# pbs-plus/pbs-plus

Measured on AMD Instinct MI355X. Metric: GiB/s ingested through CDC+SHA-256, higher is better.
Workload: dtype u32

## Files before the change

### include/pbsgpu.h

```cpp
#ifndef PBSGPU_H
#define PBSGPU_H

#include <stddef.h>
#include <stdint.h>

#ifdef __cplusplus
extern "C" {
#endif

#define PBSGPU_ABI_VERSION 5

#define PBSGPU_OK 0
#define PBSGPU_E_INVALID (-1)
#define PBSGPU_E_NO_DEVICE (-2)
#define PBSGPU_E_HIP (-3)
#define PBSGPU_E_NOMEM (-4)
#define PBSGPU_E_CAPACITY (-5)
#define PBSGPU_E_BUSY (-6)
#define PBSGPU_E_TICKET (-7)
#define PBSGPU_E_STATE (-9)

const char *pbsgpu_strerror(int status);
int pbsgpu_abi_version(void);
int pbsgpu_last_hip_error(void);
// ... 145 lines not shown
    uint32_t fill_cus;
    uint32_t reserved1;
    uint64_t reserved[2];
} pbsgpu_ring_options;
#define PBSGPU_RING_OFF 0xffffffffu
#define PBSGPU_RING_F_NO_OVERLAP 1u
#define PBSGPU_RING_F_NO_STAGE 2u
#define PBSGPU_RING_F_NO_CUT_PRIO 4u
#define PBSGPU_RING_F_NO_SPLIT_AUTO 8u
#define PBSGPU_RING_F_DEFER_SERVICE 16u
#define PBSGPU_RING_F_FILL_SERIAL 32u
#define PBSGPU_RING_F_DENSE_SERVICE 64u
#define PBSGPU_RING_F_DENSE_LANES 128u
#define PBSGPU_RING_F_TIER_TAG 256u
#define PBSGPU_RING_F_HOLD_PAGES 512u
typedef struct pbsgpu_ring_stats {
    uint64_t page_bytes, bytes_enqueued, chunks, candidates, pages_enqueued, pages_recycled, service_bytes_last;
    uint32_t pages_total, pages_free, sha_cus, rounds, rounds_done, rounds_in_flight, streams_opened, service_launches;
    double service_ms_last;
    double service_ms_total;
} pbsgpu_ring_stats;
int pbsgpu_ring_create(pbsgpu_engine *eng, const pbsgpu_ring_options *opt , pbsgpu_ring **out);
void pbsgpu_ring_destroy(pbsgpu_ring *ring);
int pbsgpu_ring_open(pbsgpu_ring *ring, uint32_t *stream);
int pbsgpu_ring_reserve(pbsgpu_ring *ring, uint32_t stream, void **dptr, uint64_t *cap);
int pbsgpu_ring_commit(pbsgpu_ring *ring, uint32_t stream, uint64_t nbytes, int final);
int pbsgpu_ring_fill(pbsgpu_ring *ring, uint32_t stream, uint64_t seed, uint32_t kind, uint64_t nbytes, int final,
                     uint64_t *taken);
typedef struct pbsgpu_fill_piece {
    uint64_t dst_off;
// ... 297 lines not shown
```

### pbs_plus_amd/_lib.py

```python
from __future__ import annotations

import ctypes as C
import os
import subprocess

import numpy as np

_HERE = os.path.dirname(os.path.abspath(__file__))
LIB_PATH = os.environ.get("PBSGPU_LIB_PATH") or os.path.join(_HERE, "lib", "libpbsgpu.so")
CSRC = os.path.join(_HERE, "csrc")

OK = 0
E_INVALID, E_NO_DEVICE, E_HIP, E_NOMEM, E_CAPACITY, E_BUSY, E_TICKET, _E_RETIRED_8, E_STATE = range(-1, -10, -1)


class PbsGpuError(RuntimeError):
    def __init__(self, status: int, what: str = ""):
        self.status = status
        msg = lib().pbsgpu_strerror(status).decode() if _lib is not None else str(status)
        hip = lib().pbsgpu_last_hip_error() if _lib is not None else 0
        extra = ""
        if _lib is not None and ("comm" in what or "allgather" in what):
            txt = lib().pbsgpu_comm_last_error()
            if txt:
# ... 44 lines not shown

class ReuseChunk(C.Structure):
    _fields_ = [("size", C.c_uint64), ("padding", C.c_uint64), ("end_offset", C.c_uint64), ("digest", C.c_uint8 * 32)]


class FileHash(C.Structure):
    _fields_ = [("index", C.c_uint64), ("size", C.c_uint64), ("xxh3", C.c_uint64)]


RING_OFF = 0xFFFFFFFF
RING_F_NO_OVERLAP, RING_F_NO_STAGE, RING_F_NO_CUT_PRIO, RING_F_NO_SPLIT_AUTO, RING_F_DEFER_SERVICE, RING_F_FILL_SERIAL = 1, 2, 4, 8, 16, 32
RING_F_DENSE_SERVICE = 64
RING_F_DENSE_LANES = 128
RING_F_TIER_TAG = 256
RING_F_HOLD_PAGES = 512
RING_ANY_STREAM = 0xFFFFFFFF


class RingOptions(C.Structure):
    _fields_ = [("arena_bytes", C.c_uint64), ("page_bytes", C.c_uint64), ("max_streams", C.c_uint32),
                ("sha_cus", C.c_uint32), ("round_pages", C.c_uint32), ("express_cus", C.c_uint32),
                ("min_round_pages", C.c_uint32), ("max_inflight", C.c_uint32), ("long_bytes", C.c_uint32),
                ("long_lo_bytes", C.c_uint32), ("long_spill", C.c_uint32), ("poll_every", C.c_uint32), ("flags", C.c_uint32),
                ("lanes_cus", C.c_uint32), ("backlog_mib", C.c_double), ("lone_defer_ms", C.c_double),
                ("idle_timeout_s", C.c_double), ("autopark_ms", C.c_double), ("short_bytes", C.c_uint64), ("fill_cus", C.c_uint32),
                ("reserved1", C.c_uint32), ("reserved", C.c_uint64 * 2)]


class EngineOptions(C.Structure):
    _fields_ = [("inflight", C.c_uint32), ("sha_form", C.c_uint32), ("sha_slack_pct", C.c_uint32), ("sha_dense_pct", C.c_uint32),
# ... 246 lines not shown
```

### pbs_plus_amd/csrc/kernels.h

```cpp
#pragma once

#include <hip/hip_runtime.h>
#include <stdint.h>

#include "../../include/pbsgpu.h"

namespace pbsk {

constexpr int kWindow = 64;

struct ScanParams {
    const uint8_t *data_al;
    uint32_t lead;
    uint64_t nbytes;
    uint64_t ntiles;
    uint32_t tile_bytes;
    const uint32_t *table_rot;
    uint32_t thr;
    uint32_t cap;
    uint32_t *tile_cnt;
    uint32_t *tile_slots;
    unsigned long long *tile_queue;
    uint32_t tiles_per_wave;
    uint32_t shared_chip;
// ... 117 lines not shown
        unsigned long long lq;
    };
    uint32_t head;
    uint32_t free_count;
    uint32_t error;
    uint32_t rounds_done;
    uint32_t xp_busy;
    uint32_t pad0;
    union {
        struct {
            uint32_t stail;
            uint32_t shead;
        };
        unsigned long long sq;
    };
    uint32_t pad[4];
};
static_assert(sizeof(RingCtl) == 64, "RingCtl is one 64-byte line");
struct RingDesc {
    uint64_t p1, p2v;
    uint32_t len, len1, cell, pages;
};
__host__ __device__ inline void ring_desc_encode(uint4 *q, const uint32_t slot, const RingDesc &d) {
    q[2u * slot] = make_uint4((uint32_t)d.p1, (uint32_t)(d.p1 >> 32), d.len, d.len1);
    q[2u * slot + 1u] = make_uint4((uint32_t)d.p2v, (uint32_t)(d.p2v >> 32), d.cell, d.pages);
}
__host__ __device__ inline RingDesc ring_desc_decode(const uint4 e0, const uint4 e1) {
    return RingDesc{((uint64_t)e0.y << 32) | e0.x, ((uint64_t)e1.y << 32) | e1.x, e0.z, e0.w, e1.z, e1.w};
}

constexpr uint32_t kCellBytes = 64;
// ... 15 lines not shown
    uint32_t smask;
    uint32_t short_bytes;
    uint32_t short_room;
    RingCtl *ctl;
    uint8_t *cells;
    uint32_t *pending;
    unsigned long long *free_fifo;
    uint32_t free_mask;
    const uint32_t *heartbeat;
    unsigned long long idle_ticks;
    uint32_t poll_mask;
    uint32_t xp;
    uint32_t long_spill;
    uint32_t xp_pairs;
    uint32_t long_lo;
};
constexpr int kHbBeat = 0, kHbIntent = 16, kHbCommitted = 17, kHbClaim = 32, kHbRoundsEnq = 33;
constexpr uint32_t kRingProbeSteps = 4096;


enum : int { kRsNcand = 0, kRsNrec = 1, kRsMaxcnt = 2, kRsNlong = 3, kRsNshort = 4, kRsShortRoom = 5, kRsTileq = 6 , kRsNmain = 8, kRsCount = 10 };

struct RingPage {
    uint64_t phys_off;
    uint64_t logical;
    uint32_t valid;
    uint32_t slot;
    uint32_t phys;
    uint32_t seg;
    uint64_t fill_seed;
    uint64_t fill_off;
// ... 107 lines not shown
```

### pbs_plus_amd/csrc/kernels.hip

```cpp
#include "kernel_util.h"
#include "kernels.h"
#include "ring_queue.h"

namespace pbsk {

__device__ __forceinline__ uint32_t rotr(uint32_t x, int n) { return __builtin_rotateright32(x, n); }

__device__ __forceinline__ uint32_t xor3(uint32_t a, uint32_t b, uint32_t c) {
    return __builtin_amdgcn_bitop3_b32(a, b, c, 0x96);
}
__device__ __forceinline__ uint32_t maj3(uint32_t a, uint32_t b, uint32_t c) {
    return __builtin_amdgcn_bitop3_b32(a, b, c, 0xE8);
}
__device__ __forceinline__ uint32_t ch3(uint32_t e, uint32_t f, uint32_t g) { return g ^ (e & (f ^ g)); }

__device__ constexpr uint32_t kSha256K[64] = {
    0x428a2f98, 0x71374491, 0xb5c0fbcf, 0xe9b5dba5, 0x3956c25b, 0x59f111f1, 0x923f82a4, 0xab1c5ed5,
    0xd807aa98, 0x12835b01, 0x243185be, 0x550c7dc3, 0x72be5d74, 0x80deb1fe, 0x9bdc06a7, 0xc19bf174,
    0xe49b69c1, 0xefbe4786, 0x0fc19dc6, 0x240ca1cc, 0x2de92c6f, 0x4a7484aa, 0x5cb0a9dc, 0x76f988da,
    0x983e5152, 0xa831c66d, 0xb00327c8, 0xbf597fc7, 0xc6e00bf3, 0xd5a79147, 0x06ca6351, 0x14292967,
    0x27b70a85, 0x2e1b2138, 0x4d2c6dfc, 0x53380d13, 0x650a7354, 0x766a0abb, 0x81c2c92e, 0x92722c85,
    0xa2bfe8a1, 0xa81a664b, 0xc24b8b70, 0xc76c51a3, 0xd192e819, 0xd6990624, 0xf40e3585, 0x106aa070,
    0x19a4c116, 0x1e376c08, 0x2748774c, 0x34b0bcb5, 0x391c0cb3, 0x4ed8aa4a, 0x5b9cca4f, 0x682e6ff3,
    0x748f82ee, 0x78a5636f, 0x84c87814, 0x8cc70208, 0x90befffa, 0xa4506ceb, 0xbef9a3f7, 0xc67178f2};
// ... 362 lines not shown
        constexpr int D = 2;
        uint32_t R[D][17];
        uint32_t selv[D], cflag[D];
        uint8_t *dstv[D];
        [[maybe_unused]] uint32_t pagesv[D];
#pragma unroll
        for (int s = 0; s < D; ++s) {
#pragma unroll
            for (int j = 0; j < 17; ++j) R[s][j] = 0;
            selv[s] = 0x00010203u;
            cflag[s] = 0;
            dstv[s] = nullptr;
            pagesv[s] = 0xffffffffu;
        }

        constexpr uint32_t kReserve = 16;
        uint32_t res_next = 0, res_end = 0;
        [[maybe_unused]] uint32_t poll_ctr = 0;
        auto acquire = [&](bool need) {
            if constexpr (Source::kRing) {
                if (__ballot(need) == 0) return;
                if (__ballot(have) != 0 && ((++poll_ctr) & src.poll_mask) != 0u) return;
                const bool long_only = src.long_bytes != 0u && src.xp == 0u && (lane & 15) == 0;
                const bool elig = need && claimed == 0u;
                if (src.long_bytes && __ballot(elig)) {
                    uint32_t lh;
                    int32_t avail = ring_queue_avail(&src.ctl->lq, lh) - (int32_t)src.long_spill;
                    if (avail > 0 && src.xp != 0u && (uint32_t)avail <= src.xp_pairs &&
                        __hip_atomic_load(&src.ctl->xp_busy, __ATOMIC_RELAXED, __HIP_MEMORY_SCOPE_AGENT) < src.xp_pairs)
                        avail = 0;
// ... 77 lines not shown
                    exhausted = true;
                    have = false;
                }
            }
            if constexpr (DENSE) {
                const uint32_t cnt = (uint32_t)__popcll(m);
                if (cnt > avail) {
                    res_next = first + (cnt - avail);
                    res_end = res_next + kReserve;
                } else {
                    res_next += cnt;
                }
            }
        };
        auto prep = [&](const int s) {
            acquire(!have && !exhausted);
            uint32_t c = 0;
            const uint8_t *p = reinterpret_cast<const uint8_t *>(kIdleBlock);
            const uint8_t *bb = base;
            uint64_t off = 0;
            bool tail = false, last = false;
            if (have) {
                off = blk * 64;
                if constexpr (Source::kRing) bb = (off < len1) ? base : base2;
                last = blk + 1 == nblk;
                if (off + 64 <= len) p = bb + off;
                else tail = true;
                c = 1u | (last ? 2u : 0u);
                dstv[s] = dst;
                if constexpr (Source::kRing) pagesv[s] = pages;
// ... 113 lines not shown
        auto rounds = [&](const Blk &x) {
            if (x.c & 1u) {
                uint32_t a = H[0], b = H[1], cc = H[2], dd = H[3], e = H[4], f = H[5], g = H[6], h = H[7];
#pragma unroll
                for (int q = 0; q < 16; q += 2) {
                    SHA256_ROUND(a, b, cc, dd, e, f, g, h, x.wk[q].x);
                    SHA256_ROUND(h, a, b, cc, dd, e, f, g, x.wk[q].y);
                    SHA256_ROUND(g, h, a, b, cc, dd, e, f, x.wk[q].z);
                    SHA256_ROUND(f, g, h, a, b, cc, dd, e, x.wk[q].w);
                    SHA256_ROUND(e, f, g, h, a, b, cc, dd, x.wk[q + 1].x);
                    SHA256_ROUND(dd, e, f, g, h, a, b, cc, x.wk[q + 1].y);
                    SHA256_ROUND(cc, dd, e, f, g, h, a, b, x.wk[q + 1].z);
                    SHA256_ROUND(b, cc, dd, e, f, g, h, a, x.wk[q + 1].w);
                }
                H[0] += a; H[1] += b; H[2] += cc; H[3] += dd; H[4] += e; H[5] += f; H[6] += g; H[7] += h;
                if (x.c & 2u) {
                    PBSK_GLOBAL uint32_t *o = (PBSK_GLOBAL uint32_t *)x.d;
#pragma unroll
                    for (int j = 0; j < 8; ++j) o[j] = __builtin_bswap32(H[j]);
                    if constexpr (Source::kRing) ring_cell_publish(o);
                    sha256_iv(H);
                }
            }
        };
        Blk A, B;
        __syncthreads();
        fetch(A, 0);
        for (;;) {
            if (!A.al) break;
            __syncthreads();
            fetch(B, 1);
            __builtin_amdgcn_sched_barrier(0);
            rounds(A);
            if (!B.al) break;
            __syncthreads();
// ... 77 lines not shown
    auto any_alive = [&](const int pb) -> uint32_t { return alive[0][pb] | alive[1][pb]; };
    for (int i = threadIdx.x; i < 2 * 2 * 2 * 16 * 32; i += 256) {
        const int row = 2 * (i & 31) + 1, q = (i >> 5) & 15, pl = (i >> 9) & 1, pb = (i >> 10) & 1, pp = (i >> 11) & 1;
        wkbuf_[pp][pb][pl][q][row] = make_uint4(1u, 1u, 1u, 1u);
    }
    __syncthreads();

    if (producer) {
        const uint32_t nitems = nitems_p ? *nitems_p : nitems_imm;
        const uint8_t *base = nullptr;
        uint64_t len = 0, blk = 0, nblk = 0;
        uint8_t *dst = nullptr;
        bool have = false, exhausted = false;
        [[maybe_unused]] const uint8_t *base2 = nullptr;
        [[maybe_unused]] uint32_t len1 = 0, pages = 0xffffffffu;
        [[maybe_unused]] unsigned long long idle_since = 0;
        [[maybe_unused]] uint32_t poll_ctr = 0;
        constexpr int D = 2;
        uint32_t R[D][17];
        uint32_t selv[D], cflag[D];
        uint8_t *dstv[D];
        [[maybe_unused]] uint32_t pagesv[D];
#pragma unroll
        for (int s = 0; s < D; ++s) {
#pragma unroll
            for (int j = 0; j < 17; ++j) R[s][j] = 0;
            selv[s] = 0x00010203u;
            cflag[s] = 0;
            dstv[s] = nullptr;
            pagesv[s] = 0xffffffffu;
        }
        auto acquire = [&](bool need) {
            if (__ballot(need) == 0) return;
            bool got = false;
            if constexpr (Source::kRing) {
                if (__ballot(have) != 0 && ((++poll_ctr) & src.poll_mask) != 0u) return;
                uint32_t lh;
                const int32_t avail = ring_queue_avail(&src.ctl->lq, lh);
                const unsigned long long mn = __ballot(need);
                if (avail > 0) {
                    const uint32_t cnt = min((uint32_t)__popcll(mn), (uint32_t)avail);
                    const uint32_t first = ring_cas_claim(&src.ctl->lhead, lh, cnt, mn, lane);
                    if (first != 0xffffffffu) {
                        const uint32_t rank = wave_rank(mn, lane);
                        got = need && rank < cnt;
                        uint4 e0, e1;
                        ring_desc_load(src.ldesc, (first + rank) & src.lmask, got, e0, e1);
                        ring_desc_take(src, got, e0, e1, base, base2, len, len1, dst, pages);
                        if (lane == __ffsll((long long)mn) - 1) atomicAdd(&src.ctl->xp_busy, cnt);
                    }
                } else if (ring_stop_raised(src) && ring_drained_after_stop(&src.ctl->lq)) {
                    exhausted = exhausted | need;
                }
            } else {
                const unsigned long long m = __ballot(need);
                const uint32_t first = wave_claim(queue, m, (uint32_t)__popcll(m), lane);
                if (need) {
                    const uint32_t i = first + wave_rank(m, lane);
                    if (i < nitems) {
                        src.get(i, base, len, dst);
                        got = true;
                    } else {
                        exhausted = true;
                    }
                }
            }
            const int srcl = lane & ~1;
// ... 9 lines not shown
                    dst = reinterpret_cast<uint8_t *>(ds);
                }
                if constexpr (Source::kRing) {
                    const uint64_t b2 = (uint64_t)__shfl((unsigned long long)reinterpret_cast<uintptr_t>(base2), srcl, 64);
                    const uint32_t l1 = (uint32_t)__shfl((int)len1, srcl, 64);
                    const uint32_t pg = (uint32_t)__shfl((int)pages, srcl, 64);
                    if (pgot) {
                        base2 = reinterpret_cast<const uint8_t *>(b2);
                        len1 = l1;
                        pages = pg;
                    }
                }
                if (pgot) {
                    nblk = (len + 8) / 64 + 1;
                    blk = roleB ? 1ull : 0ull;
                    have = blk < nblk;
                }
            }
        };
        auto prep = [&](const int s) {
            const unsigned long long hm = __ballot(have);
            const bool pair_busy = ((hm >> (lane & ~1)) & 3ull) != 0ull;
            acquire(!roleB && !pair_busy && !exhausted);
            uint32_t c = 0;
            const uint8_t *p = reinterpret_cast<const uint8_t *>(kIdleBlock);
            const uint8_t *bb = base;
            uint64_t off = 0;
            bool tail = false, last = false;
            if (have) {
                off = blk * 64;
                if constexpr (Source::kRing) bb = (off < len1) ? base : base2;
                last = blk + 1 == nblk;
                if (off + 64 <= len) p = bb + off;
                else tail = true;
                c = 1u | (last ? 2u : 0u);
                dstv[s] = dst;
                if constexpr (Source::kRing) pagesv[s] = pages;
                blk += 2;
                if (blk >= nblk) have = false;
            }
            sha256_request_block(p, R[s], selv[s]);
            if (tail) {
                sha256_tail_words(bb, len, off, last, R[s]);
                selv[s] = 0x00010203u;
            }
            cflag[s] = c;
        };
        const int wrow = lane & ~1, wplane = lane & 1;

#pragma unroll
        for (int s = 0; s < D; ++s) prep(s);
        bool drained = false;
// ... 63 lines not shown
        uint32_t HR[4] = {ivr[0], ivr[1], ivr[2], ivr[3]};
        struct Blk {
            uint32_t al, c;
            uint8_t *d;
            uint4 wk[16];
        };
        auto fetch = [&](Blk &x, const int pb, const int plane) {
            x.al = any_alive(pb);
            x.c = ctrl[pb][plane][ci];
            x.d = dstp[pb][plane][ci];
#pragma unroll
            for (int q = 0; q < 16; ++q) x.wk[q] = wkbuf[pb][plane][q][lane];
        };
        auto rounds = [&](const Blk &x) {
            if (x.c & 1u) {
                uint32_t x0 = xp_sel(role, HR[0], HR[2]), x1 = xp_sel(role, HR[1], HR[3]), x2 = HR[2], x3 = HR[3];
                xp_round4<true>(x0, x1, x2, x3, x.wk[0], R, HR[1], HR[0]);
#pragma unroll
                for (int g = 1; g < 16; ++g) xp_round4<false>(x0, x1, x2, x3, x.wk[g], R);
                const uint32_t o63 = x0, o62 = x1, o61 = x2, o60 = x3;
                xp_round2(x0, x1, x2, x3, x.wk[15].w, R);
                HR[0] += xp_sel(role, o63, x0);
                HR[1] += xp_sel(role, o62, x1);
                HR[2] += xp_sel(role, o61, o63);
                HR[3] += xp_sel(role, o60, o62);
                if (x.c & 2u) {
                    PBSK_GLOBAL uint32_t *o = (PBSK_GLOBAL uint32_t *)x.d + (roleB ? 0 : 4);
#pragma unroll
                    for (int j = 0; j < 4; ++j) o[j] = __builtin_bswap32(HR[j]);
                    if constexpr (Source::kRing) ring_cell_publish((PBSK_GLOBAL uint32_t *)x.d);
// ... 207 lines not shown
```

### pbs_plus_amd/csrc/ring.cpp

```cpp
#include <chrono>
#include <cstdio>
#include <cstdlib>
#include <thread>

#include "ring_internal.h"

using namespace pbse;

namespace {

double now_ms() {
    return std::chrono::duration<double, std::milli>(std::chrono::steady_clock::now().time_since_epoch()).count();
}

volatile uint32_t *hb_words(const pbsgpu_ring *r) { return r->heartbeat.as<volatile uint32_t>(); }

void ring_service_ended(pbsgpu_ring *r) {
    if (r->svc == SvcState::Stopped) return;
    r->svc = SvcState::Stopped;
    float ms = 0;
    if (hipEventElapsedTime(&ms, r->ev_svc0, r->ev_svc1) == hipSuccess) {
        r->st.service_ms_last = ms;
        r->st.service_ms_total += ms;
    } else {
// ... 477 lines not shown
        {"PBSGPU_RING_LONG_SPILL", U32, &o.long_spill, 0},
        {"PBSGPU_RING_POLL_EVERY", U32, &o.poll_every, 0},
        {"PBSGPU_RING_BACKLOG_MIB", F64_ZERO_NEG, &o.backlog_mib, 0},
        {"PBSGPU_RING_LONE_DEFER_MS", F64_ZERO_NEG, &o.lone_defer_ms, 0},
        {"PBSGPU_RING_IDLE_TIMEOUT_S", F64, &o.idle_timeout_s, 0},
        {"PBSGPU_RING_AUTOPARK_MS", F64, &o.autopark_ms, 0},
        {"PBSGPU_RING_OVERLAP", FLAG_IF_ZERO, &o.flags, PBSGPU_RING_F_NO_OVERLAP},
        {"PBSGPU_RING_STAGE_INPUTS", FLAG_IF_ZERO, &o.flags, PBSGPU_RING_F_NO_STAGE},
        {"PBSGPU_RING_CUT_PRIO", FLAG_IF_ZERO, &o.flags, PBSGPU_RING_F_NO_CUT_PRIO},
        {"PBSGPU_RING_SPLIT_AUTO", FLAG_IF_ZERO, &o.flags, PBSGPU_RING_F_NO_SPLIT_AUTO},
        {"PBSGPU_RING_DEFER_SERVICE", FLAG_IF_SET, &o.flags, PBSGPU_RING_F_DEFER_SERVICE},
        {"PBSGPU_RING_FILL_SERIAL", FLAG_IF_SET, &o.flags, PBSGPU_RING_F_FILL_SERIAL},
        {"PBSGPU_RING_DENSE_SERVICE", FLAG_IF_SET, &o.flags, PBSGPU_RING_F_DENSE_SERVICE},
        {"PBSGPU_RING_DENSE_LANES", FLAG_IF_SET, &o.flags, PBSGPU_RING_F_DENSE_LANES},
        {"PBSGPU_RING_TIER_TAG", FLAG_IF_SET, &o.flags, PBSGPU_RING_F_TIER_TAG},
    };
    for (const Entry &e : table) {
        const char *v = getenv(e.name);
        if (!v || !*v) continue;
        switch (e.kind) {
        case U32: *static_cast<uint32_t *>(e.field) = (uint32_t)std::max(0L, atol(v)); break;
        case U32_ZERO_OFF: *static_cast<uint32_t *>(e.field) = atol(v) <= 0 ? PBSGPU_RING_OFF : (uint32_t)atol(v); break;
        case U64: *static_cast<uint64_t *>(e.field) = strtoull(v, nullptr, 10); break;
        case F64: *static_cast<double *>(e.field) = std::max(0.0, atof(v)); break;
        case F64_ZERO_NEG: *static_cast<double *>(e.field) = atof(v) <= 0.0 ? -1.0 : atof(v); break;
        case FLAG_IF_ZERO: if (atoi(v) == 0) *static_cast<uint32_t *>(e.field) |= e.flag; break;
        case FLAG_IF_SET: if (atoi(v) != 0) *static_cast<uint32_t *>(e.field) |= e.flag; break;
        }
    }
}
// ... 15 lines not shown
    const pbsp::QueuePolicy pol = pbsp::queue_policy({lanes_cus, xp_cus, dense_lanes, long_lo_auto, long_bytes, opt_long_lo,
                                                      opt_long_spill, opt_poll_every, idle_timeout_s, eng->cfg.max,
                                                      std::min(eng->effmin, eng->cfg.min)});
    q.short_room = pol.short_room;
    q.xp_pairs = pol.xp_pairs;
    q.long_spill = pol.long_spill;
    q.long_lo = pol.long_lo;
    q.idle_ticks = pol.idle_ticks;
    q.poll_mask = pol.poll_mask;
    q.ctl = ctl.as<pbsk::RingCtl>();
    q.cells = cells.as<uint8_t>();
    q.pending = pending.as<uint32_t>();
    q.free_fifo = free_fifo.as<unsigned long long>();
    q.free_mask = nfree - 1;
    q.heartbeat = heartbeat.as<uint32_t>();
    return q;
}

namespace pbse {

void ring_pop_records(pbsgpu_ring *r, uint32_t slot, pbsgpu_record *out, uint64_t cap, uint64_t *n) {
    StreamSlot &s = r->slots[slot];
    const uint8_t *cells = r->cells.as<uint8_t>();
    while (*n < cap && !s.cells.empty()) {
        const CellRef cr = s.cells.front();
        const uint8_t *c = cells + (size_t)cr.cell * pbsk::kCellBytes;
        const volatile uint32_t *cw = reinterpret_cast<const volatile uint32_t *>(c);
        if (cw[pbsk::kCellFlag] != 1u) break;
        std::atomic_thread_fence(std::memory_order_acquire);
        pbsgpu_record rec;
// ... 102 lines not shown
    r->opt_fill_cus = o.fill_cus;
    r->stage_inputs = !(o.flags & PBSGPU_RING_F_NO_STAGE);
    return PBSGPU_OK;
}

static int ring_allocate(pbsgpu_ring *r, bool overlap) {
    const uint64_t ntiles = r->ntiles;
    CHK(r->arena.ensure((size_t)r->npages * r->stride + 512));
    CHK(r->ctl.ensure(256));
    CHK(r->probe.ensure(128));
    CHK(r->streams.ensure((size_t)r->max_streams * sizeof(pbsk::RingStreamState)));
    CHK(r->pending.ensure((size_t)r->npages * 4 + 64));
    CHK(r->desc.ensure((size_t)r->qslots * 32));
    CHK(r->ldesc.ensure((size_t)r->lslots * 32));
    CHK(r->sdesc.ensure((size_t)r->sslots * 32));
    CHK(r->scalars.ensure(pbsk::kRsCount * 4 + 64));
    CHK(r->tile_cnt.ensure((size_t)ntiles * 4 + 16));
    CHK(r->tile_off.ensure((size_t)ntiles * 4 + 16));
    CHK(r->tile_slots.ensure((size_t)ntiles * r->cap * 4 + 16));
    CHK(r->tileq.ensure(128 + kRingInputs * 8));
    if (overlap) {
        CHK(r->tile_cnt2.ensure((size_t)ntiles * 4 + 16));
        CHK(r->tile_slots2.ensure((size_t)ntiles * r->cap * 4 + 16));
    }
    CHK(r->dense.ensure((size_t)r->dense_cap * 8 + 16));
    CHK(r->scan_tmp.ensure(pbsk::scan_tmp_words(std::max<uint64_t>(ntiles, r->max_streams)) * 4 + 64));
    CHK(r->segs.ensure((size_t)r->max_streams * sizeof(pbsgpu_segment)));
    CHK(r->seg_cnt.ensure((size_t)r->max_streams * 4 + 16));
    CHK(r->seg_off.ensure((size_t)r->max_streams * 4 + 16));
    CHK(r->seg_newc.ensure((size_t)r->max_streams * 8 + 16));
// ... 15 lines not shown
    r->input_stride = r->in_status_off + 128;
    CHK(r->inputs.ensure(r->input_stride * kRingInputs));
    if (r->stage_inputs) CHK(r->inputs_dev.ensure(r->input_stride * kRingInputs));
    std::memset(r->inputs.p, 0, r->input_stride * kRingInputs);
    return PBSGPU_OK;
}

static int ring_streams_and_events(pbsgpu_ring *r, bool overlap, bool cut_prio) {
    int prio_lo = 0, prio_hi = 0;
    HIPCHK(hipDeviceGetStreamPriorityRange(&prio_lo, &prio_hi));
    r->bulk_prio = cut_prio ? prio_lo : 0;
    HIPCHK(hipStreamCreateWithFlags(&r->cs, hipStreamNonBlocking));
    HIPCHK(hipStreamCreateWithPriority(&r->fs, hipStreamNonBlocking, r->bulk_prio));
    HIPCHK(hipMemsetAsync(r->ctl.p, 0, 256, r->cs));
    HIPCHK(hipMemsetAsync(r->probe.p, 0, 128, r->cs));
    HIPCHK(hipMemsetAsync(r->streams.p, 0, (size_t)r->max_streams * sizeof(pbsk::RingStreamState), r->cs));
    HIPCHK(hipMemsetAsync(r->pending.p, 0, (size_t)r->npages * 4 + 64, r->cs));
    HIPCHK(hipMemsetAsync(r->scalars.p, 0, pbsk::kRsCount * 4 + 64, r->cs));
    HIPCHK(hipMemsetAsync(r->tileq.p, 0, 128 + kRingInputs * 8, r->cs));
    HIPCHK(hipStreamSynchronize(r->cs));
    for (auto &ev : r->ev_fill) HIPCHK(hipEventCreateWithFlags(&ev, hipEventDisableTiming));
    if (overlap) {
        HIPCHK(hipStreamCreateWithPriority(&r->ps, hipStreamNonBlocking, r->bulk_prio));
        for (auto &ev : r->ev_scan) HIPCHK(hipEventCreateWithFlags(&ev, hipEventDisableTiming));
        for (auto &ev : r->ev_ctl) HIPCHK(hipEventCreateWithFlags(&ev, hipEventDisableTiming));
    }
    HIPCHK(hipStreamCreateWithPriority(&r->ss, hipStreamNonBlocking, prio_hi));
    if (r->xp_cus) {
        HIPCHK(hipStreamCreateWithPriority(&r->xs, hipStreamNonBlocking, prio_hi));
        HIPCHK(hipEventCreateWithFlags(&r->ev_xsvc1, hipEventDisableTiming));
// ... 23 lines not shown
    r->eng = e;
    const bool overlap = !(o.flags & PBSGPU_RING_F_NO_OVERLAP);
    int st = ring_shape(r, o, long_bytes_hint);
    if (st == PBSGPU_OK) st = ring_allocate(r, overlap);
    if (st == PBSGPU_OK) st = ring_streams_and_events(r, overlap, !(o.flags & PBSGPU_RING_F_NO_CUT_PRIO));
    if (st != PBSGPU_OK) {
        pbsgpu_ring_destroy(r);
        return st;
    }
    r->slots.resize(r->max_streams);
    r->piece_tab.resize(r->max_streams);
    r->piece_n.assign(r->max_streams, 0);
    r->free_pages.reserve(r->npages);
    for (uint32_t p = r->npages; p-- > 0;) r->free_pages.push_back(p);
    r->hold = (o.flags & PBSGPU_RING_F_HOLD_PAGES) != 0;
    if (r->hold) r->held.init(r->npages, r->max_streams, r->page_bytes);
    r->st.pages_total = r->npages;
    r->st.page_bytes = r->page_bytes;
    r->st.sha_cus = r->sha_cus;
    *out = r;
    return PBSGPU_OK;
}

}

extern "C" {

int pbsgpu_ring_create(pbsgpu_engine *e, const pbsgpu_ring_options *opt, pbsgpu_ring **out) {
    return ring_create_internal(e, opt, true, out);
}
// ... 64 lines not shown
        if (r->fs) (void)hipStreamDestroy(r->fs);
        for (auto ev : r->ev_scan)
            if (ev) (void)hipEventDestroy(ev);
        for (auto ev : r->ev_ctl)
            if (ev) (void)hipEventDestroy(ev);
        for (auto ev : r->ev_fill)
            if (ev) (void)hipEventDestroy(ev);
        for (hipEvent_t ev : {r->ev_reset, r->ev_svc0, r->ev_svc1})
            if (ev) (void)hipEventDestroy(ev);
        for (auto &s : r->slots)
            for (auto &q : s.ready)
                if (q.dep) r->ev_pool.push_back(q.dep);
        for (auto ev : r->ev_pool) (void)hipEventDestroy(ev);
        for (DevBuf *b : {&r->arena, &r->ctl, &r->probe, &r->streams, &r->pending, &r->desc, &r->ldesc, &r->sdesc, &r->scalars, &r->tile_cnt, &r->tile_off,
                          &r->tile_slots, &r->tile_cnt2, &r->tile_slots2, &r->tileq, &r->scan_tmp, &r->dense, &r->segs, &r->seg_cnt, &r->seg_off, &r->recs, &r->seg_newc,
                          &r->seg_open, &r->seg_ecand_in, &r->seg_ecand, &r->inputs_dev})
            b->release();
        r->cells.release();
        r->heartbeat.release();
        r->free_fifo.release();
        r->inputs.release();
        for (auto &b : r->sugg_in) b.release();
        for (auto &b : r->piece_tab) b.release();
    }
    const bool unref = r->holds_engine_ref;
    delete r;
    if (e && unref) engine_unref(e);
}

int pbsgpu_ring_open(pbsgpu_ring *r, uint32_t *stream) {
    if (!r || !stream) return PBSGPU_E_INVALID;
// ... 454 lines not shown
        const StreamSlot &s = r->slots[i];
        if (!s.open) continue;
        put("stream %u: committed=%llu enqueued=%llu final_committed=%d final_enqueued=%d final_done=%d ready=%zu cells=%zu "
            "out=%llu | device c=%llu end=%llu\n", i, (unsigned long long)s.bytes_committed,
            (unsigned long long)s.bytes_enqueued, (int)s.final_committed, (int)s.final_enqueued, (int)s.final_done,
            s.ready.size(), s.cells.size(), (unsigned long long)s.records_out, (unsigned long long)sts[i].c,
            (unsigned long long)sts[i].end);
        if (!s.cells.empty()) {
            const uint8_t *c = r->cells.as<uint8_t>() + (size_t)s.cells.front().cell * pbsk::kCellBytes;
            pbsgpu_record rec;
            std::memcpy(&rec, c, sizeof(rec));
            put("  waiting for cell %u: end=%llu size=%u flag=%u\n", s.cells.front().cell, (unsigned long long)rec.end, rec.size,
                reinterpret_cast<const uint32_t *>(c)[pbsk::kCellFlag]);
        }
    }
    return PBSGPU_OK;
}

int pbsgpu_ring_express(pbsgpu_ring *r, uint32_t *express_cus, uint64_t *long_bytes) {
    if (!r) return PBSGPU_E_INVALID;
    if (express_cus) *express_cus = r->xp_cus;
    if (long_bytes) *long_bytes = r->xp_cus ? r->long_bytes : 0;
    return PBSGPU_OK;
}

int pbsgpu_ring_get_probe(pbsgpu_ring *r, pbsgpu_ring_probe *out) {
    if (!r || !out) return PBSGPU_E_INVALID;
    static_assert(sizeof(pbsgpu_ring_probe) == 48, "six counters");
    if (r->svc == SvcState::Running) {
        ring_reap_rounds(r);
// ... 24 lines not shown
```

### pbs_plus_amd/csrc/ring_internal.h

```cpp
#pragma once

#include <deque>
#include <mutex>
#include <vector>

#include "engine_internal.h"
#include "hold.h"
#include "ring_plan.h"

namespace pbse {

constexpr uint32_t kRingInputs = 16;
constexpr uint32_t kPagesPerStreamRound = 256;

struct PageReq {
    uint32_t phys = 0;
    uint64_t k = 0;
    uint32_t valid = 0;
    bool final = false;
    bool do_fill = false;
    uint64_t seed = 0, fill_off = 0;
    uint32_t kind = 0;
    const pbsk::FillPiece *tab = nullptr;
    uint32_t ntab = 0;
// ... 37 lines not shown
    uint64_t new_bytes = 0;
};

enum class SvcState { Stopped, Running, Stopping };

}

struct pbsgpu_ring : pbsp::RingShape {
    pbsgpu_engine *eng = nullptr;
    bool holds_engine_ref = true;
    std::mutex mu;
    uint64_t ready_bytes = 0, inflight_bytes = 0;
    uint32_t tail_seen = 0;
    uint64_t pub_positions = 0, pub_bytes = 0;
    pbse::DevBuf arena, ctl, streams, pending, desc, ldesc, sdesc, probe;
    unsigned long long probe_seen[6] = {};
    bool probe_seen_valid = false;
    unsigned long long ctl_phase_ticks[2][5] = {};
    unsigned long long ctl_phase_rounds[2] = {};
    pbse::DevBuf scalars, tile_cnt, tile_off, tile_slots, scan_tmp, dense, segs, seg_cnt, seg_off, recs, seg_newc, seg_open;
    pbse::DevBuf tile_cnt2, tile_slots2, tileq;
    pbse::DevBuf seg_ecand_in, seg_ecand;
    pbse::DevBuf inputs_dev;
    bool stage_inputs = true;
    pbse::PinnedBuf cells, free_fifo, inputs, heartbeat;
    std::vector<pbse::PinnedBuf> piece_tab;
    std::vector<uint32_t> piece_n;
    pbse::PinnedBuf sugg_in[pbse::kRingInputs];
    size_t input_stride = 0, in_pages_off = 0, in_segs_off = 0, in_recbase_off = 0, in_suggidx_off = 0, in_status_off = 0;
    hipStream_t cs = nullptr, ss = nullptr, fs = nullptr;
// ... 102 lines not shown
```

### pbs_plus_amd/csrc/ring_plan.h

```cpp
#pragma once

#include <algorithm>
#include <cstddef>
#include <cstdint>
#include <cstdlib>

#include "../../include/pbsgpu.h"

namespace pbsp {

inline uint32_t pow2_at_least(uint64_t v) {
    uint32_t p = 1;
    while (p < v && p < (1u << 31)) p <<= 1;
    return p;
}

struct ChunkerView {
    uint32_t min, effmin, avg, max, mask;
    uint32_t minsz() const { return std::min(effmin, min); }
};

inline uint64_t seg_cell_bound(uint32_t take, uint64_t page_bytes, uint32_t maxsz, uint32_t minsz) {
    return ((uint64_t)take * page_bytes + maxsz) / minsz + 2;
}
// ... 187 lines not shown
    q.long_lo = (v.xp_cus && v.long_lo_auto) ? (uint32_t)((uint64_t)v.cfg_max * 11 / 16) : 0u;
    if (v.opt_long_lo) q.long_lo = (v.xp_cus && v.opt_long_lo != PBSGPU_RING_OFF) ? v.opt_long_lo : 0u;
    if (q.long_lo >= v.long_bytes) q.long_lo = 0u;
    if (v.opt_long_spill) q.long_spill = v.opt_long_spill;
    const double idle_s = v.idle_timeout_s > 0 ? std::max(0.05, v.idle_timeout_s) : 20.0;
    q.idle_ticks = (unsigned long long)(idle_s * 100e6);
    {
        const uint64_t min_steps = v.minsz / 64u;
        int every = (int)std::min<uint64_t>(64, std::max<uint64_t>(8, pow2_at_least(min_steps / 256u + 1u) / 2u));
        if (v.opt_poll_every) every = (int)v.opt_poll_every;
        q.poll_mask = pow2_at_least((uint64_t)every) - 1u;
    }
    return q;
}

}
```

### pbs_plus_amd/csrc/ring_queue.h

```cpp
#pragma once

#include "kernel_util.h"
#include "kernels.h"

namespace pbsk {


__device__ __forceinline__ uint32_t wave_rank(const unsigned long long m, const int lane) {
    return (uint32_t)__popcll(m & ((1ull << lane) - 1ull));
}

__device__ __forceinline__ uint32_t wave_claim(uint32_t *queue, const unsigned long long m, const uint32_t n, const int lane) {
    uint32_t first = 0;
    const int leader = __ffsll((long long)m) - 1;
    if (lane == leader) first = atomicAdd(queue, n);
    return __shfl(first, leader, 64);
}

__device__ __forceinline__ int32_t ring_queue_avail(const unsigned long long *q, uint32_t &head) {
    const unsigned long long v = __hip_atomic_load(q, __ATOMIC_RELAXED, __HIP_MEMORY_SCOPE_AGENT);
    head = (uint32_t)(v >> 32);
    return (int32_t)((uint32_t)v - head);
}

// ... 25 lines not shown
    len = take ? (uint64_t)d.len : len;
    len1 = take ? d.len1 : len1;
    dst = take ? src.cells + (uint64_t)d.cell * kCellBytes + 4u * kCellDigest : dst;
    pages = take ? d.pages : pages;
}

__device__ __forceinline__ bool ring_drained_after_stop(const unsigned long long *q) {
    __atomic_thread_fence(__ATOMIC_ACQUIRE);
    uint32_t h;
    return ring_queue_avail(q, h) <= 0;
}
__device__ __forceinline__ bool ring_stop_raised(const RingSource &src) {
    return (uint32_t)(__hip_atomic_load(&src.ctl->tail_stop, __ATOMIC_RELAXED, __HIP_MEMORY_SCOPE_AGENT) >> 32) != 0u;
}

__device__ __forceinline__ void ring_report_free(const RingSource &q, const uint32_t page) {
    const uint32_t fs = atomicAdd(&q.ctl->free_count, 1u);
    __hip_atomic_store(&q.free_fifo[fs & q.free_mask], ((unsigned long long)(fs + 1u) << 32) | page, __ATOMIC_RELAXED,
                       __HIP_MEMORY_SCOPE_SYSTEM);
}
__device__ __forceinline__ void ring_release_page(const RingSource &q, const uint32_t page) {
    if (__hip_atomic_fetch_sub(&q.pending[page], 1u, __ATOMIC_RELEASE, __HIP_MEMORY_SCOPE_AGENT) == 1u) ring_report_free(q, page);
}
__device__ __forceinline__ void ring_release_pages(const RingSource &q, const uint32_t pages) {
#pragma unroll
    for (int h = 0; h < 2; ++h) {
        const uint32_t pi = h ? (pages >> 16) : (pages & 0xffffu);
        if (pi != 0xffffu) ring_release_page(q, pi);
    }
}
// ... 8 lines not shown
```

Baseline: 708.7.

## Hand over long in-progress SHA chunks from lane workers to idle express pairs

Adds a continuation queue so single-lane SHA workers can periodically offer a long chunk still in progress, saving their intermediate hash state and remaining descriptor into a cont slot. Idle express-pair (xp) workers claim these entries, reload the saved state and finish the chunk with the faster two-lane path. The aim is to cut tail latency from long chunks that are stuck on slow lanes while xp capacity sits idle. In exchange it adds atomics, fences, extra per-block flag checks and new termination conditions, which raises ordering and correctness risk. It is on by default and can be turned off with a new flag or environment variable.

```diff
diff --git a/include/pbsgpu.h b/include/pbsgpu.h
--- a/include/pbsgpu.h
+++ b/include/pbsgpu.h
@@ -183,6 +183,7 @@
 #define PBSGPU_RING_F_DENSE_LANES 128u
 #define PBSGPU_RING_F_TIER_TAG 256u
 #define PBSGPU_RING_F_HOLD_PAGES 512u
+#define PBSGPU_RING_F_NO_HANDOVER 1024u
 typedef struct pbsgpu_ring_stats {
     uint64_t page_bytes, bytes_enqueued, chunks, candidates, pages_enqueued, pages_recycled, service_bytes_last;
     uint32_t pages_total, pages_free, sha_cus, rounds, rounds_done, rounds_in_flight, streams_opened, service_launches;
diff --git a/pbs_plus_amd/_lib.py b/pbs_plus_amd/_lib.py
--- a/pbs_plus_amd/_lib.py
+++ b/pbs_plus_amd/_lib.py
@@ -82,6 +82,7 @@
 RING_F_DENSE_LANES = 128
 RING_F_TIER_TAG = 256
 RING_F_HOLD_PAGES = 512
+RING_F_NO_HANDOVER = 1024
 RING_ANY_STREAM = 0xFFFFFFFF
 
 
diff --git a/pbs_plus_amd/csrc/kernels.h b/pbs_plus_amd/csrc/kernels.h
--- a/pbs_plus_amd/csrc/kernels.h
+++ b/pbs_plus_amd/csrc/kernels.h
@@ -155,7 +155,15 @@
         };
         unsigned long long sq;
     };
-    uint32_t pad[4];
+    union {
+        struct {
+            uint32_t ctail;
+            uint32_t chead;
+        };
+        unsigned long long cq;
+    };
+    uint32_t cinfl;
+    uint32_t pad[1];
 };
 static_assert(sizeof(RingCtl) == 64, "RingCtl is one 64-byte line");
 struct RingDesc {
@@ -201,7 +209,14 @@
     uint32_t long_spill;
     uint32_t xp_pairs;
     uint32_t long_lo;
-};
+    uint8_t *cont;
+    uint32_t cmask;
+    uint32_t ho_min;
+};
+constexpr uint32_t kContBytes = 128;
+enum : uint32_t { kContDesc = 0, kContState = 8, kContBlk = 16, kContReady = 17 };
+__host__ __device__ inline uint32_t ring_cont_tag(const uint32_t ticket) { return (ticket & 0x07ffffffu) + 1u; }
+enum : uint32_t { kBlkValid = 1u, kBlkLast = 2u, kBlkHand = 4u, kBlkTagShift = 4u };
 constexpr int kHbBeat = 0, kHbIntent = 16, kHbCommitted = 17, kHbClaim = 32, kHbRoundsEnq = 33;
 constexpr uint32_t kRingProbeSteps = 4096;
 
diff --git a/pbs_plus_amd/csrc/kernels.hip b/pbs_plus_amd/csrc/kernels.hip
--- a/pbs_plus_amd/csrc/kernels.hip
+++ b/pbs_plus_amd/csrc/kernels.hip
@@ -400,6 +400,30 @@
             pagesv[s] = 0xffffffffu;
         }
 
+        [[maybe_unused]] uint32_t ho_left = 1, ho_period = 1;
+        if constexpr (Source::kRing && !DENSE) {
+            ho_period = 8u * (src.poll_mask + 1u);
+            asm volatile("" : "+v"(ho_period));
+        }
+        auto offer = [&](const int s) {
+            if constexpr (Source::kRing && !DENSE) {
+                const int o = s ^ 1;
+                const bool cand = src.ho_min != 0u && have && nblk - blk >= (uint64_t)src.ho_min &&
+                                  (cflag[o] & (kBlkValid | kBlkLast)) == kBlkValid;
+                const unsigned long long m = __ballot(cand);
+                uint32_t room = 0;
+                if (m != 0ull) room = ring_cont_room(src);
+                const uint32_t cnt = min((uint32_t)__popcll(m), room);
+                uint32_t first = 0xffffffffu;
+                if (cnt != 0u) first = ring_cont_reserve(src, cnt, m, lane);
+                const uint32_t ticket = first + wave_rank(m, lane);
+                const bool push = cand && first != 0xffffffffu && wave_rank(m, lane) < cnt;
+                if (push) ring_cont_write(src, ticket, base, base2, (uint32_t)len, len1, dst, pages, (uint32_t)blk);
+                if (__ballot(push)) __builtin_amdgcn_fence(__ATOMIC_RELEASE, "agent");
+                cflag[o] = push ? (cflag[o] | kBlkHand | (ring_cont_tag(ticket) << kBlkTagShift)) : cflag[o];
+                have = have && !push;
+            }
+        };
         constexpr uint32_t kReserve = 16;
         uint32_t res_next = 0, res_end = 0;
         [[maybe_unused]] uint32_t poll_ctr = 0;
@@ -507,6 +531,16 @@
             }
         };
         auto prep = [&](const int s) {
+            if constexpr (Source::kRing && !DENSE) {
+                if (s == 0) {
+                    ho_left -= 1u;
+                    asm volatile("" : "+v"(ho_left));
+                    if (__builtin_amdgcn_readfirstlane(ho_left) == 0u) {
+                        ho_left = ho_period;
+                        offer(s);
+                    }
+                }
+            }
             acquire(!have && !exhausted);
             uint32_t c = 0;
             const uint8_t *p = reinterpret_cast<const uint8_t *>(kIdleBlock);
@@ -650,11 +684,24 @@
                     SHA256_ROUND(b, cc, dd, e, f, g, h, a, x.wk[q + 1].w);
                 }
                 H[0] += a; H[1] += b; H[2] += cc; H[3] += dd; H[4] += e; H[5] += f; H[6] += g; H[7] += h;
-                if (x.c & 2u) {
+                constexpr bool kHands = Source::kRing && !DENSE;
+                if (x.c & (kHands ? (kBlkLast | kBlkHand) : kBlkLast)) {
                     PBSK_GLOBAL uint32_t *o = (PBSK_GLOBAL uint32_t *)x.d;
-#pragma unroll
-                    for (int j = 0; j < 8; ++j) o[j] = __builtin_bswap32(H[j]);
-                    if constexpr (Source::kRing) ring_cell_publish(o);
+                    bool hand = false;
+                    if constexpr (kHands) hand = (x.c & kBlkHand) != 0u;
+                    if (hand) {
+                        if constexpr (kHands) {
+                            const uint32_t tag = x.c >> kBlkTagShift;
+                            PBSK_GLOBAL uint32_t *st = ring_cont_entry(src, tag - 1u) + kContState;
+#pragma unroll
+                            for (int j = 0; j < 8; ++j) st[j] = H[j];
+                            ring_cont_publish(st, tag);
+                        }
+                    } else {
+#pragma unroll
+                        for (int j = 0; j < 8; ++j) o[j] = __builtin_bswap32(H[j]);
+                        if constexpr (Source::kRing) ring_cell_publish(o);
+                    }
                     sha256_iv(H);
                 }
             }
@@ -762,6 +809,7 @@
         bool have = false, exhausted = false;
         [[maybe_unused]] const uint8_t *base2 = nullptr;
         [[maybe_unused]] uint32_t len1 = 0, pages = 0xffffffffu;
+        [[maybe_unused]] uint8_t *cont_st = nullptr;
         [[maybe_unused]] unsigned long long idle_since = 0;
         [[maybe_unused]] uint32_t poll_ctr = 0;
         constexpr int D = 2;
@@ -781,6 +829,8 @@
         auto acquire = [&](bool need) {
             if (__ballot(need) == 0) return;
             bool got = false;
+            [[maybe_unused]] uint32_t first_blk = 0;
+            [[maybe_unused]] uint8_t *from_cont = nullptr;
             if constexpr (Source::kRing) {
                 if (__ballot(have) != 0 && ((++poll_ctr) & src.poll_mask) != 0u) return;
                 uint32_t lh;
@@ -797,8 +847,21 @@
                         ring_desc_take(src, got, e0, e1, base, base2, len, len1, dst, pages);
                         if (lane == __ffsll((long long)mn) - 1) atomicAdd(&src.ctl->xp_busy, cnt);
                     }
-                } else if (ring_stop_raised(src) && ring_drained_after_stop(&src.ctl->lq)) {
-                    exhausted = exhausted | need;
+                } else {
+                    uint32_t ccnt = 0;
+                    const uint32_t cfirst = src.ho_min ? ring_cont_claim(src, need, mn, lane, ccnt) : 0xffffffffu;
+                    if (cfirst != 0xffffffffu) {
+                        const uint32_t rank = wave_rank(mn, lane);
+                        got = need && rank < ccnt;
+                        uint4 e0, e1;
+                        ring_cont_load(src, cfirst + rank, got, e0, e1, first_blk);
+                        ring_desc_take(src, got, e0, e1, base, base2, len, len1, dst, pages);
+                        from_cont = got ? src.cont + (uint64_t)((cfirst + rank) & src.cmask) * kContBytes + 4u * kContState : from_cont;
+                        ring_cont_taken(src, ccnt, mn, lane);
+                    } else if (ring_stop_raised(src) && ring_drained_after_stop(&src.ctl->lq) &&
+                               (src.ho_min == 0u || ring_cont_none_left(src))) {
+                        exhausted = exhausted | need;
+                    }
                 }
             } else {
                 const unsigned long long m = __ballot(need);
@@ -838,6 +901,10 @@
                 if (pgot) {
                     nblk = (len + 8) / 64 + 1;
                     blk = roleB ? 1ull : 0ull;
+                    if constexpr (Source::kRing) {
+                        blk += (uint64_t)(uint32_t)__shfl((int)first_blk, srcl, 64);
+                        cont_st = roleB ? nullptr : from_cont;
+                    }
                     have = blk < nblk;
                 }
             }
@@ -859,7 +926,12 @@
                 else tail = true;
                 c = 1u | (last ? 2u : 0u);
                 dstv[s] = dst;
-                if constexpr (Source::kRing) pagesv[s] = pages;
+                if constexpr (Source::kRing) {
+                    pagesv[s] = pages;
+                    c |= cont_st ? kBlkHand : 0u;
+                    dstv[s] = cont_st ? cont_st : dst;
+                    cont_st = nullptr;
+                }
                 blk += 2;
                 if (blk >= nblk) have = false;
             }
@@ -953,6 +1025,13 @@
         };
         auto rounds = [&](const Blk &x) {
             if (x.c & 1u) {
+                if constexpr (Source::kRing) {
+                    if (x.c & kBlkHand) {
+                        PBSK_GLOBAL uint32_t *st = (PBSK_GLOBAL uint32_t *)x.d + (roleB ? 0 : 4);
+#pragma unroll
+                        for (int j = 0; j < 4; ++j) HR[j] = __hip_atomic_load(st + j, __ATOMIC_RELAXED, __HIP_MEMORY_SCOPE_AGENT);
+                    }
+                }
                 uint32_t x0 = xp_sel(role, HR[0], HR[2]), x1 = xp_sel(role, HR[1], HR[3]), x2 = HR[2], x3 = HR[3];
                 xp_round4<true>(x0, x1, x2, x3, x.wk[0], R, HR[1], HR[0]);
 #pragma unroll
diff --git a/pbs_plus_amd/csrc/ring.cpp b/pbs_plus_amd/csrc/ring.cpp
--- a/pbs_plus_amd/csrc/ring.cpp
+++ b/pbs_plus_amd/csrc/ring.cpp
@@ -515,6 +515,7 @@
         {"PBSGPU_RING_DENSE_SERVICE", FLAG_IF_SET, &o.flags, PBSGPU_RING_F_DENSE_SERVICE},
         {"PBSGPU_RING_DENSE_LANES", FLAG_IF_SET, &o.flags, PBSGPU_RING_F_DENSE_LANES},
         {"PBSGPU_RING_TIER_TAG", FLAG_IF_SET, &o.flags, PBSGPU_RING_F_TIER_TAG},
+        {"PBSGPU_RING_HANDOVER", FLAG_IF_ZERO, &o.flags, PBSGPU_RING_F_NO_HANDOVER},
     };
     for (const Entry &e : table) {
         const char *v = getenv(e.name);
@@ -560,6 +561,9 @@
     q.free_fifo = free_fifo.as<unsigned long long>();
     q.free_mask = nfree - 1;
     q.heartbeat = heartbeat.as<uint32_t>();
+    q.cont = cont.as<uint8_t>();
+    q.cmask = cont_slots ? cont_slots - 1 : 0;
+    q.ho_min = (handover && xp_cus && cont_slots && !dense_service) ? pbsp::handover_min_blocks(eng->cfg.max) : 0u;
     return q;
 }
 
@@ -692,6 +696,10 @@
     CHK(r->desc.ensure((size_t)r->qslots * 32));
     CHK(r->ldesc.ensure((size_t)r->lslots * 32));
     CHK(r->sdesc.ensure((size_t)r->sslots * 32));
+    if (r->xp_cus) {
+        r->cont_slots = pbsp::handover_slots(r->svc_cus);
+        CHK(r->cont.ensure((size_t)r->cont_slots * pbsk::kContBytes));
+    }
     CHK(r->scalars.ensure(pbsk::kRsCount * 4 + 64));
     CHK(r->tile_cnt.ensure((size_t)ntiles * 4 + 16));
     CHK(r->tile_off.ensure((size_t)ntiles * 4 + 16));
@@ -737,6 +745,7 @@
     HIPCHK(hipStreamCreateWithPriority(&r->fs, hipStreamNonBlocking, r->bulk_prio));
     HIPCHK(hipMemsetAsync(r->ctl.p, 0, 256, r->cs));
     HIPCHK(hipMemsetAsync(r->probe.p, 0, 128, r->cs));
+    if (r->cont_slots) HIPCHK(hipMemsetAsync(r->cont.p, 0, (size_t)r->cont_slots * pbsk::kContBytes, r->cs));
     HIPCHK(hipMemsetAsync(r->streams.p, 0, (size_t)r->max_streams * sizeof(pbsk::RingStreamState), r->cs));
     HIPCHK(hipMemsetAsync(r->pending.p, 0, (size_t)r->npages * 4 + 64, r->cs));
     HIPCHK(hipMemsetAsync(r->scalars.p, 0, pbsk::kRsCount * 4 + 64, r->cs));
@@ -790,6 +799,7 @@
     r->free_pages.reserve(r->npages);
     for (uint32_t p = r->npages; p-- > 0;) r->free_pages.push_back(p);
     r->hold = (o.flags & PBSGPU_RING_F_HOLD_PAGES) != 0;
+    r->handover = !(o.flags & PBSGPU_RING_F_NO_HANDOVER);
     if (r->hold) r->held.init(r->npages, r->max_streams, r->page_bytes);
     r->st.pages_total = r->npages;
     r->st.page_bytes = r->page_bytes;
@@ -884,7 +894,7 @@
         for (auto ev : r->ev_pool) (void)hipEventDestroy(ev);
         for (DevBuf *b : {&r->arena, &r->ctl, &r->probe, &r->streams, &r->pending, &r->desc, &r->ldesc, &r->sdesc, &r->scalars, &r->tile_cnt, &r->tile_off,
                           &r->tile_slots, &r->tile_cnt2, &r->tile_slots2, &r->tileq, &r->scan_tmp, &r->dense, &r->segs, &r->seg_cnt, &r->seg_off, &r->recs, &r->seg_newc,
-                          &r->seg_open, &r->seg_ecand_in, &r->seg_ecand, &r->inputs_dev})
+                          &r->seg_open, &r->seg_ecand_in, &r->seg_ecand, &r->inputs_dev, &r->cont})
             b->release();
         r->cells.release();
         r->heartbeat.release();
@@ -1369,6 +1379,11 @@
                 reinterpret_cast<const uint32_t *>(c)[pbsk::kCellFlag]);
         }
     }
+    {
+        unsigned long long pr[16] = {};
+        HIPCHK(hipMemcpy(pr, r->probe.p, sizeof(pr), hipMemcpyDeviceToHost));
+        put("handover: pushed=%llu taken=%llu in_flight=%u min_blocks=%u\n", pr[10], pr[11], ctl.cinfl, r->source().ho_min);
+    }
     return PBSGPU_OK;
 }
 
diff --git a/pbs_plus_amd/csrc/ring_internal.h b/pbs_plus_amd/csrc/ring_internal.h
--- a/pbs_plus_amd/csrc/ring_internal.h
+++ b/pbs_plus_amd/csrc/ring_internal.h
@@ -75,6 +75,9 @@
     uint32_t tail_seen = 0;
     uint64_t pub_positions = 0, pub_bytes = 0;
     pbse::DevBuf arena, ctl, streams, pending, desc, ldesc, sdesc, probe;
+    pbse::DevBuf cont;
+    uint32_t cont_slots = 0;
+    bool handover = true;
     unsigned long long probe_seen[6] = {};
     bool probe_seen_valid = false;
     unsigned long long ctl_phase_ticks[2][5] = {};
diff --git a/pbs_plus_amd/csrc/ring_plan.h b/pbs_plus_amd/csrc/ring_plan.h
--- a/pbs_plus_amd/csrc/ring_plan.h
+++ b/pbs_plus_amd/csrc/ring_plan.h
@@ -225,4 +225,8 @@
     return q;
 }
 
-}
+constexpr uint32_t kBlockFifoDepth = 2;
+inline uint32_t handover_min_blocks(uint32_t cfg_max) { return std::max<uint32_t>(kBlockFifoDepth + 2u, cfg_max / 64u / 2u); }
+inline uint32_t handover_slots(uint32_t svc_cus) { return pow2_at_least((uint64_t)std::max(1u, svc_cus) * 64u); }
+
+}
diff --git a/pbs_plus_amd/csrc/ring_queue.h b/pbs_plus_amd/csrc/ring_queue.h
--- a/pbs_plus_amd/csrc/ring_queue.h
+++ b/pbs_plus_amd/csrc/ring_queue.h
@@ -63,6 +63,95 @@
     return (uint32_t)(__hip_atomic_load(&src.ctl->tail_stop, __ATOMIC_RELAXED, __HIP_MEMORY_SCOPE_AGENT) >> 32) != 0u;
 }
 
+__device__ __forceinline__ PBSK_GLOBAL uint32_t *ring_cont_entry(const RingSource &q, const uint32_t ticket) {
+    return (PBSK_GLOBAL uint32_t *)(q.cont + (uint64_t)(ticket & q.cmask) * kContBytes);
+}
+__device__ __forceinline__ uint32_t ring_cont_limit(const RingSource &q) { return min(q.xp_pairs, q.cmask + 1u); }
+
+__device__ __forceinline__ uint32_t ring_cont_room(const RingSource &q) {
+    const unsigned long long ts = __hip_atomic_load(&q.ctl->tail_stop, __ATOMIC_RELAXED, __HIP_MEMORY_SCOPE_AGENT);
+    const uint32_t hd = __hip_atomic_load(&q.ctl->head, __ATOMIC_RELAXED, __HIP_MEMORY_SCOPE_AGENT);
+    const uint32_t xb = __hip_atomic_load(&q.ctl->xp_busy, __ATOMIC_RELAXED, __HIP_MEMORY_SCOPE_AGENT);
+    const uint32_t ci = __hip_atomic_load(&q.ctl->cinfl, __ATOMIC_RELAXED, __HIP_MEMORY_SCOPE_AGENT);
+    uint32_t lh;
+    const int32_t la = ring_queue_avail(&q.ctl->lq, lh);
+    const uint32_t lim = ring_cont_limit(q);
+    if ((uint32_t)(ts >> 32) != 0u || (int32_t)(hd - (uint32_t)ts) < 0 || la > 0 || xb + ci >= lim) return 0u;
+    return lim - xb - ci;
+}
+
+__device__ __forceinline__ uint32_t ring_cont_reserve(const RingSource &q, const uint32_t cnt, const unsigned long long m, const int lane) {
+    const int leader = __ffsll((long long)m) - 1;
+    uint32_t first = 0xffffffffu;
+    if (lane == leader) {
+        const uint32_t prev = atomicAdd(&q.ctl->cinfl, cnt);
+        __builtin_amdgcn_fence(__ATOMIC_SEQ_CST, "agent");
+        if (ring_stop_raised(q) || prev + cnt > ring_cont_limit(q)) {
+            atomicSub(&q.ctl->cinfl, cnt);
+        } else {
+            first = atomicAdd(&q.ctl->ctail, cnt);
+            if (q.probe) atomicAdd(q.probe + 10, (unsigned long long)cnt);
+        }
+    }
+    return __shfl(first, leader, 64);
+}
+
+__device__ __forceinline__ void ring_cont_write(const RingSource &q, const uint32_t ticket, const uint8_t *base, const uint8_t *base2,
+                                                const uint32_t len, const uint32_t len1, const uint8_t *dst, const uint32_t pages,
+                                                const uint32_t blk) {
+    PBSK_GLOBAL uint32_t *e = ring_cont_entry(q, ticket);
+    const uint64_t p1 = (uint64_t)reinterpret_cast<uintptr_t>(base), p2 = (uint64_t)reinterpret_cast<uintptr_t>(base2);
+    const uint32_t cell = (uint32_t)((uint64_t)(dst - q.cells - 4u * kCellDigest) / kCellBytes);
+    PBSK_GLOBAL u32x4_a4 *d = (PBSK_GLOBAL u32x4_a4 *)(e + kContDesc);
+    d[0] = u32x4_a4{(uint32_t)p1, (uint32_t)(p1 >> 32), len, len1};
+    d[1] = u32x4_a4{(uint32_t)p2, (uint32_t)(p2 >> 32), cell, pages};
+    e[kContBlk] = blk;
+}
+__device__ __forceinline__ void ring_cont_load(const RingSource &q, const uint32_t ticket, const bool pred, uint4 &e0, uint4 &e1,
+                                               uint32_t &blk) {
+    e0 = make_uint4(0, 0, 0, 0);
+    e1 = make_uint4(0, 0, 0, 0);
+    if (pred) {
+        const PBSK_GLOBAL uint32_t *e = ring_cont_entry(q, ticket);
+        const u32x4_a4 v0 = ((gvec4_ptr)(e + kContDesc))[0], v1 = ((gvec4_ptr)(e + kContDesc))[1];
+        e0 = make_uint4(v0.x, v0.y, v0.z, v0.w);
+        e1 = make_uint4(v1.x, v1.y, v1.z, v1.w);
+        blk = e[kContBlk];
+    }
+}
+
+__device__ __forceinline__ void ring_cont_publish(PBSK_GLOBAL uint32_t *st, const uint32_t tag) {
+    __builtin_amdgcn_fence(__ATOMIC_RELEASE, "agent");
+    __hip_atomic_store(st + (kContReady - kContState), tag, __ATOMIC_RELAXED, __HIP_MEMORY_SCOPE_AGENT);
+}
+
+__device__ __forceinline__ uint32_t ring_cont_claim(const RingSource &q, const bool need, const unsigned long long mn, const int lane,
+                                                    uint32_t &cnt) {
+    uint32_t ch;
+    const int32_t avail = ring_queue_avail(&q.ctl->cq, ch);
+    cnt = 0;
+    if (avail <= 0) return 0xffffffffu;
+    const uint32_t rank = wave_rank(mn, lane);
+    bool ready = false;
+    if (need && rank < (uint32_t)avail)
+        ready = __hip_atomic_load(ring_cont_entry(q, ch + rank) + kContReady, __ATOMIC_RELAXED, __HIP_MEMORY_SCOPE_AGENT) ==
+                ring_cont_tag(ch + rank);
+    const unsigned long long bad = __ballot(need && !ready);
+    cnt = (uint32_t)__popcll(bad ? (mn & ((1ull << (__ffsll((long long)bad) - 1)) - 1ull)) : mn);
+    if (cnt == 0) return 0xffffffffu;
+    return ring_cas_claim(&q.ctl->chead, ch, cnt, mn, lane);
+}
+__device__ __forceinline__ void ring_cont_taken(const RingSource &q, const uint32_t cnt, const unsigned long long mn, const int lane) {
+    __builtin_amdgcn_fence(__ATOMIC_RELEASE, "agent");
+    if (lane != __ffsll((long long)mn) - 1) return;
+    atomicAdd(&q.ctl->xp_busy, cnt);
+    atomicSub(&q.ctl->cinfl, cnt);
+    if (q.probe) atomicAdd(q.probe + 11, (unsigned long long)cnt);
+}
+__device__ __forceinline__ bool ring_cont_none_left(const RingSource &q) {
+    return __hip_atomic_load(&q.ctl->cinfl, __ATOMIC_RELAXED, __HIP_MEMORY_SCOPE_AGENT) == 0u;
+}
+
 __device__ __forceinline__ void ring_report_free(const RingSource &q, const uint32_t page) {
     const uint32_t fs = atomicAdd(&q.ctl->free_count, 1u);
     __hip_atomic_store(&q.free_fifo[fs & q.free_mask], ((unsigned long long)(fs + 1u) << 32) | page, __ATOMIC_RELAXED,
```

After: 710.2 (median of 2 runs). About the same (+0.2%).
